# Mirko-Nava/BayesianNeuralNetworks

Measured on AMD Instinct MI355X. Metric: MC-samples/sec (node), 784-1200-1200-10 BayesianLinear MLP, batch 512, higher is better.
Workload: dtype bf16; 1 GPU; configs[1]: MNIST-shape 784-1200-1200-10 NormalLinear MLP, batch 512, 8 MC samples per forward per GPU (8 in all), KL once per forward, predictive mean; bf16 operands / fp32 accumulate; batch=512, hip_graph=True

## Files before the change

### bayesianneuralnetworks_amd/csrc/bnn_dense.hip

```cpp
#include <cstdlib>
#include <type_traits>

#include "bnn_device.hpp"
#include "bnn_dma.hpp"
#include "bnn_kl_body.hpp"

namespace bnn {

typedef float f32x4 __attribute__((ext_vector_type(4)));
typedef __bf16 bf16x8 __attribute__((ext_vector_type(8)));

constexpr int kDrawMaxTensors = 8;
constexpr int kDrawSpreadBelow = 4096;

struct DrawTensorDev {
    const float *mu;
    const float *rho;
    void *out;
    int64_t out_sample_stride;
    int32_t rows, cols, ld;
    int32_t bf16;
    int32_t kind;
    int32_t perm_taps;
    int32_t first_item;
// ... 207 lines not shown
        s_lo = local / nit;
        local -= s_lo * nit;
        s_hi = s_lo < S ? s_lo + 1 : 0;
        s_step = 1;
    }
    if (t_kind == 3) {
        if (L.t[ti].spread ? s_lo != 0 : blockIdx.y != 0) return;
        s_lo = 0; s_hi = 1; s_step = 1;
    }
    const int row = local / gpr, c0 = (local - row * gpr) << 3;
    if (row >= t_rows) return;
    const int64_t orow = (int64_t)row * t_ld + c0;
    const int esz = t_bf16 ? 2 : 4;
    char *const dst0 = t_out + orow * esz;
    const int64_t sbytes = t_stride * esz;
    const int64_t pbytes = sbytes * (t_kind == 3 ? 1 : L.nsamples);
    if (!LEAN && t_kind == BNN_DRAW_FLIPOUT) {
        float m[8], sg[8];
#pragma unroll
        for (int j = 0; j < 8; ++j) {
            const bool v = c0 + j < t_cols;
            m[j] = v ? t_mu[(int64_t)row * t_cols + c0 + j] : 0.f;
            sg[j] = v ? sigma_draw(t_rho[(int64_t)row * t_cols + c0 + j]) : 0.f;
        }
        const uint32_t edev = rng_epoch_dev(rng);
        const uint32_t e0 = (uint32_t)t_rows + (uint32_t)c0, q0 = e0 >> 2, off = e0 & 3u;
#pragma unroll 1
        for (int s = s_lo; s < s_hi; s += s_step) {
            const uint32_t sample = rng.sample0 + (uint32_t)s;
            const float r = flip_sign(drop_u1(rng, edev, (uint32_t)row, sample));
            const float4 ua = drop_u4(rng, edev, q0, sample), ub = drop_u4(rng, edev, q0 + 1u, sample), uc = drop_u4(rng, edev, q0 + 2u, sample);
            const float u[12] = {ua.x, ua.y, ua.z, ua.w, ub.x, ub.y, ub.z, ub.w, uc.x, uc.y, uc.z, uc.w};
            float w[8];
#pragma unroll
            for (int j = 0; j < 8; ++j) {
                const float uj = off == 0u ? u[j] : off == 1u ? u[j + 1] : off == 2u ? u[j + 2] : u[j + 3];
                w[j] = fmaf(sg[j], r * flip_sign(uj), m[j]);
            }
            char *dst = dst0 + (int64_t)s * sbytes;
            if (t_bf16) {
                uint4 o;
                o.x = pack_bf16x2(w[0], w[1]); o.y = pack_bf16x2(w[2], w[3]);
                o.z = pack_bf16x2(w[4], w[5]); o.w = pack_bf16x2(w[6], w[7]);
                *reinterpret_cast<uint4 *>(dst) = o;
            } else {
#pragma unroll
                for (int j = 0; j < 8; ++j)
                    if (c0 + j < t_ld) reinterpret_cast<float *>(dst)[j] = w[j];
            }
        }
        return;
    }
    const bool regular = t_bf16 && t_kind == 0 && t_taps <= 1 && (t_cols & 7) == 0 &&
                         (((reinterpret_cast<uintptr_t>(t_mu) | reinterpret_cast<uintptr_t>(t_rho)) & 15u) == 0);
    if (regular) {
        const bool pad = c0 >= t_cols;
        const int64_t e0 = pad ? 0 : (int64_t)row * t_cols + c0;
        const uint32_t edev = rng_epoch_dev(rng);
        const float4 m0 = *reinterpret_cast<const float4 *>(t_mu + e0), m1 = *reinterpret_cast<const float4 *>(t_mu + e0 + 4);
        const float4 r0 = *reinterpret_cast<const float4 *>(t_rho + e0), r1 = *reinterpret_cast<const float4 *>(t_rho + e0 + 4);
        const float live = pad ? 0.f : 1.f;
        const float m[8] = {pad ? 0.f : m0.x, pad ? 0.f : m0.y, pad ? 0.f : m0.z, pad ? 0.f : m0.w,
                            pad ? 0.f : m1.x, pad ? 0.f : m1.y, pad ? 0.f : m1.z, pad ? 0.f : m1.w};
        const float sg[8] = {live * sigma_draw(r0.x), live * sigma_draw(r0.y), live * sigma_draw(r0.z), live * sigma_draw(r0.w),
                             live * sigma_draw(r1.x), live * sigma_draw(r1.y), live * sigma_draw(r1.z), live * sigma_draw(r1.w)};
        const PhiloxKeys keys = philox_keys(rng.key0, rng.key1);
        const uint32_t blk = (uint32_t)(e0 >> 2);
        char *dst = dst0 + (int64_t)s_lo * sbytes;
        const int64_t step = sbytes * (int64_t)s_step;
        const bool gen16 = LEAN || rng.gen == BNN_GEN_PHILOX7_U16;
#pragma unroll U
        for (int s = s_lo; s < s_hi; s += s_step, dst += step) {
            const uint32_t sample = rng.sample0 + (uint32_t)s;
            float4 za, zb;
            if (gen16) {
                eps8_u16(rng, keys, edev, blk >> 1, sample, za, zb);
            } else {
                za = eps4(rng, keys, edev, blk, sample);
                zb = eps4(rng, keys, edev, blk + 1u, sample);
            }
            float w[8];
            w[0] = fmaf(sg[0], za.x, m[0]); w[1] = fmaf(sg[1], za.y, m[1]);
            w[2] = fmaf(sg[2], za.z, m[2]); w[3] = fmaf(sg[3], za.w, m[3]);
            w[4] = fmaf(sg[4], zb.x, m[4]); w[5] = fmaf(sg[5], zb.y, m[5]);
            w[6] = fmaf(sg[6], zb.z, m[6]); w[7] = fmaf(sg[7], zb.w, m[7]);
            if (t_x3) {
                uint4 h, mm, l;
                split_bf16x3(w[0], w[1], h.x, mm.x, l.x); split_bf16x3(w[2], w[3], h.y, mm.y, l.y);
                split_bf16x3(w[4], w[5], h.z, mm.z, l.z); split_bf16x3(w[6], w[7], h.w, mm.w, l.w);
                *reinterpret_cast<uint4 *>(dst) = h;
                *reinterpret_cast<uint4 *>(dst + pbytes) = mm;
                *reinterpret_cast<uint4 *>(dst + 2 * pbytes) = l;
            } else {
                uint4 o;
                o.x = pack_bf16x2(w[0], w[1]); o.y = pack_bf16x2(w[2], w[3]);
                o.z = pack_bf16x2(w[4], w[5]); o.w = pack_bf16x2(w[6], w[7]);
                *reinterpret_cast<uint4 *>(dst) = o;
            }
        }
        return;
    }
    if (LEAN) {
        const int64_t e0 = (int64_t)row * t_cols + c0;
        const int nval = c0 >= t_cols ? 0 : t_cols - c0 < 8 ? t_cols - c0 : 8;
        float m[8], sg[8];
#pragma unroll
        for (int j = 0; j < 8; ++j) {
            const bool v = j < nval;
            m[j] = v ? (t_kind != 2 ? t_mu[e0 + j] : sigma_accurate(t_rho[e0 + j])) : 0.f;
            sg[j] = v && t_kind == 0 ? sigma_draw(t_rho[e0 + j]) : 0.f;
        }
        const uint32_t edev = rng_epoch_dev(rng);
        const uint32_t blk = (uint32_t)(e0 >> 2);
        for (int s = s_lo; s < s_hi; s += s_step) {
            const uint32_t sample = rng.sample0 + (uint32_t)s;
            float4 za = make_float4(0.f, 0.f, 0.f, 0.f), zb = za;
            if (t_kind == 0) {
                za = eps4_u16(rng, edev, blk, sample);
                zb = eps4_u16(rng, edev, blk + 1u, sample);
            }
            float w[8];
            w[0] = fmaf(sg[0], za.x, m[0]); w[1] = fmaf(sg[1], za.y, m[1]);
            w[2] = fmaf(sg[2], za.z, m[2]); w[3] = fmaf(sg[3], za.w, m[3]);
            w[4] = fmaf(sg[4], zb.x, m[4]); w[5] = fmaf(sg[5], zb.y, m[5]);
            w[6] = fmaf(sg[6], zb.z, m[6]); w[7] = fmaf(sg[7], zb.w, m[7]);
#pragma unroll
            for (int j = 0; j < 8; ++j) w[j] = j < nval ? w[j] : 0.f;
            char *dst = dst0 + s * sbytes;
            if (t_bf16) {
                uint4 o;
                o.x = pack_bf16x2(w[0], w[1]); o.y = pack_bf16x2(w[2], w[3]);
                o.z = pack_bf16x2(w[4], w[5]); o.w = pack_bf16x2(w[6], w[7]);
                *reinterpret_cast<uint4 *>(dst) = o;
            } else {
#pragma unroll
                for (int j = 0; j < 8; ++j)
                    if (c0 + j < t_ld) reinterpret_cast<float *>(dst)[j] = w[j];
            }
        }
        return;
    }
    if (c0 >= t_cols) {
        for (int s = s_lo; s < s_hi; s += s_step) {
            if (t_bf16) {
                for (int pl = 0; pl < (t_x3 ? 3 : 1); ++pl) *reinterpret_cast<uint4 *>(dst0 + s * sbytes + pl * pbytes) = make_uint4(0u, 0u, 0u, 0u);
            } else
                for (int j = 0; j < 8; ++j)
                    if (c0 + j < t_ld) reinterpret_cast<float *>(dst0 + s * sbytes)[j] = 0.f;
        }
        return;
    }
    const int64_t e0 = (int64_t)row * t_cols + c0;
    const int nval = t_cols - c0 < 8 ? t_cols - c0 : 8;
    const bool full = nval == 8 && (((reinterpret_cast<uintptr_t>(t_mu) | reinterpret_cast<uintptr_t>(t_rho)) & 15u) == 0) && (e0 & 3) == 0;
    float m[8], sg[8];
    if (t_kind != 0) {
#pragma unroll
        for (int j = 0; j < 8; ++j) {
            m[j] = j < nval ? (t_kind != 2 ? t_mu[e0 + j] : sigma_accurate(t_rho[e0 + j])) : 0.f;
            sg[j] = 0.f;
        }
    } else if (full) {
        const float4 m0 = *reinterpret_cast<const float4 *>(t_mu + e0), m1 = *reinterpret_cast<const float4 *>(t_mu + e0 + 4);
        const float4 r0 = *reinterpret_cast<const float4 *>(t_rho + e0), r1 = *reinterpret_cast<const float4 *>(t_rho + e0 + 4);
        m[0] = m0.x; m[1] = m0.y; m[2] = m0.z; m[3] = m0.w; m[4] = m1.x; m[5] = m1.y; m[6] = m1.z; m[7] = m1.w;
        sg[0] = sigma_draw(r0.x); sg[1] = sigma_draw(r0.y); sg[2] = sigma_draw(r0.z); sg[3] = sigma_draw(r0.w);
        sg[4] = sigma_draw(r1.x); sg[5] = sigma_draw(r1.y); sg[6] = sigma_draw(r1.z); sg[7] = sigma_draw(r1.w);
    } else {
#pragma unroll
        for (int j = 0; j < 8; ++j) {
            m[j] = j < nval ? t_mu[e0 + j] : 0.f;
            sg[j] = j < nval ? sigma_draw(t_rho[e0 + j]) : 0.f;
        }
    }
    const uint32_t edev = rng_epoch_dev(rng);
    const PhiloxKeys keys = philox_keys(rng.key0, rng.key1);
    const uint32_t blk = (uint32_t)(e0 >> 2);
    const bool vec_store = t_bf16 && nval == 8 && t_taps <= 1;
#pragma unroll U
    for (int s = s_lo; s < s_hi; s += s_step) {
        const uint32_t sample = rng.sample0 + (uint32_t)s;
        float4 za = make_float4(0.f, 0.f, 0.f, 0.f), zb = za;
        if (LEAN && t_kind == 0) {
            za = eps4_u16(rng, keys, edev, blk, sample);
            zb = eps4_u16(rng, keys, edev, blk + 1u, sample);
        } else if (t_kind == 0) {
            za = eps4(rng, keys, edev, blk, sample);
            zb = eps4(rng, keys, edev, blk + 1u, sample);
        }
        float w[8];
        w[0] = fmaf(sg[0], za.x, m[0]); w[1] = fmaf(sg[1], za.y, m[1]);
        w[2] = fmaf(sg[2], za.z, m[2]); w[3] = fmaf(sg[3], za.w, m[3]);
        w[4] = fmaf(sg[4], zb.x, m[4]); w[5] = fmaf(sg[5], zb.y, m[5]);
        w[6] = fmaf(sg[6], zb.z, m[6]); w[7] = fmaf(sg[7], zb.w, m[7]);
        char *dst = dst0 + s * sbytes;
        if (vec_store && t_x3) {
            uint4 h, m, l;
            split_bf16x3(w[0], w[1], h.x, m.x, l.x); split_bf16x3(w[2], w[3], h.y, m.y, l.y);
            split_bf16x3(w[4], w[5], h.z, m.z, l.z); split_bf16x3(w[6], w[7], h.w, m.w, l.w);
            *reinterpret_cast<uint4 *>(dst) = h;
            *reinterpret_cast<uint4 *>(dst + pbytes) = m;
            *reinterpret_cast<uint4 *>(dst + 2 * pbytes) = l;
        } else if (vec_store) {
            uint4 o;
            o.x = pack_bf16x2(w[0], w[1]); o.y = pack_bf16x2(w[2], w[3]);
            o.z = pack_bf16x2(w[4], w[5]); o.w = pack_bf16x2(w[6], w[7]);
            *reinterpret_cast<uint4 *>(dst) = o;
        } else if (!LEAN && t_taps > 1) {
            const int Cn = t_cols / t_taps;
            uint16_t *rowp = reinterpret_cast<uint16_t *>(t_out + ((int64_t)row * t_ld) * 2 + s * sbytes);
            for (int j = 0; j < nval; ++j) {
                const int col = c0 + j, c = col / t_taps, tp = col - c * t_taps;
                if (t_x3) {
                    uint32_t h, m, l;
                    split_bf16x3(w[j], 0.f, h, m, l);
                    rowp[tp * Cn + c] = (uint16_t)h;
                    *reinterpret_cast<uint16_t *>(reinterpret_cast<char *>(rowp + tp * Cn + c) + pbytes) = (uint16_t)m;
                    *reinterpret_cast<uint16_t *>(reinterpret_cast<char *>(rowp + tp * Cn + c) + 2 * pbytes) = (uint16_t)l;
                } else
                    rowp[tp * Cn + c] = f2bf(w[j]);
            }
            for (int j = nval; j < 8 && c0 + j < t_ld; ++j)
                for (int pl = 0; pl < (t_x3 ? 3 : 1); ++pl)
                    *reinterpret_cast<uint16_t *>(reinterpret_cast<char *>(rowp + c0 + j) + pl * pbytes) = 0;
        } else {
            for (int j = 0; j < 8; ++j) {
                if (c0 + j >= t_ld) break;
                const float v = j < nval ? w[j] : 0.f;
                if (t_x3) {
                    uint32_t h, m, l;
                    split_bf16x3(v, 0.f, h, m, l);
                    reinterpret_cast<uint16_t *>(dst)[j] = (uint16_t)h;
                    reinterpret_cast<uint16_t *>(dst + pbytes)[j] = (uint16_t)m;
                    reinterpret_cast<uint16_t *>(dst + 2 * pbytes)[j] = (uint16_t)l;
                } else if (t_bf16) reinterpret_cast<uint16_t *>(dst)[j] = f2bf(v);
                else reinterpret_cast<float *>(dst)[j] = v;
            }
        }
    }
}

struct DenseParams {
    const uint16_t *A;
    int64_t a_sample_stride;
    int64_t lda;
    const uint16_t *W;
    int64_t w_sample_stride;
    int64_t ldw;
    const float *bias;
    int64_t bias_sample_stride;
    void *Y;
    int64_t y_sample_stride;
    int64_t ldy;
    int32_t M, N, K, S;
    int32_t ntm, ntn;
    int32_t flags;
    int32_t x3;
    int64_t a_plane_stride, w_plane_stride, y_plane_stride;
    const uint16_t *Wh;
    int64_t wh_sample_stride, ldwh;
    const float *bias_h;
    int64_t bias_h_sample_stride;
    float *P;
    int32_t Nh;
    int64_t wh_plane_stride;
    RngDev drop_rng;
    float drop_p, drop_scale;
    int32_t drop_fan;
};

constexpr int kDenseLoaderPrio = 1 << 21;
constexpr int kDenseNoXcdMap = 1 << 20;

__device__ __forceinline__ void dma_piece(const void *base, uint32_t voff, uint32_t lds)
{
    uint32_t keep;
    asm volatile("s_mov_b32 %0, m0\n\ts_mov_b32 m0, %3\n\ts_nop 0\n\tglobal_load_lds_dwordx4 %1, %2\n\ts_mov_b32 m0, %0"
                 : "=&s"(keep) : "v"(voff), "s"(base), "s"(lds) : "memory");
}

template <int TM, int TN, int NWM, int NWN, int ST, int YM, bool RELU, int DIAG = 0, bool DROP = false>
__global__ __launch_bounds__(512, ST == 2 ? 4 : 1) void k_dense_bf16(const DenseParams p)
{
    static_assert(!DROP || YM <= 1, "the dropout epilogue stores fp32 or bf16");
    constexpr bool CO = ST == 2;
    constexpr int NWV = 4;
    constexpr bool INTERLEAVE = true;
    constexpr int MPR = DIAG == 3 ? 1 : DIAG == 4 ? 2 : TN >= 8 ? 2 : 1;
    static_assert(NWM * NWN == NWV, "four consumer waves");
    constexpr int WM = 16 * TM, WN = 16 * TN, BM = NWM * WM, BN = NWN * WN;
    constexpr int A_TOTAL = BM / 8;
    constexpr int B_TOTAL = BN / 8;
    static_assert(A_TOTAL % NWV == 0, "A pieces divide evenly over the loaders");
    constexpr int A_PIECES = A_TOTAL / NWV;
    constexpr int B_BASE = B_TOTAL / NWV, B_EXTRA = B_TOTAL % NWV;
    constexpr int A_STAGE = BM * 128;
    constexpr int B_STAGE = BN * 128;
    constexpr int STAGE = A_STAGE + B_STAGE;
    constexpr bool YBF = YM != 0;
    constexpr int ESZ = YBF ? 2 : 4;
    constexpr int EPI_BYTES = ST * STAGE / NWV;
    constexpr int EPI_A = (EPI_BYTES / (16 * (WN * ESZ + 16))) < TM ? (EPI_BYTES / (16 * (WN * ESZ + 16))) : TM;
    static_assert(EPI_A >= 1, "a quarter of the ring must hold at least 16 output rows (epilogue staging)");
    __shared__ __attribute__((aligned(16))) char lds[ST * STAGE];

    const int per_s = p.ntm * p.ntn;
    int s, t;
    {
        const int L = (int)blockIdx.x;
        if (p.flags & kDenseNoXcdMap) {
            s = L / per_s;
            t = L % per_s;
        } else if (p.S % 8 == 0) {
            const int idx = L >> 3;
            s = (L & 7) + 8 * (idx / per_s);
            t = idx % per_s;
        } else {
            const int total = per_s * p.S, x = L & 7;
            const int u = x * (total >> 3) + (x < (total & 7) ? x : (total & 7)) + (L >> 3);
            s = u / per_s;
            t = u % per_s;
        }
    }
    int mt, panel;
    if (per_s > 32 && !(p.flags & kDenseNoXcdMap)) {
        constexpr int GM = 4;
        const int grp = t / (GM * p.ntn), first = grp * GM;
        const int gm = p.ntm - first < GM ? p.ntm - first : GM;
        const int v = t - grp * (GM * p.ntn);
        mt = first + v % gm;
        panel = v / gm;
    } else {
        mt = t / p.ntn;
        panel = t % p.ntn;
    }
    const int m0 = mt * BM, n0 = panel * BN;
    const int tid = threadIdx.x, lane = tid & 63;
    const int wave = __builtin_amdgcn_readfirstlane(tid >> 6);
    const int nk = (p.K + 63) / 64 * (p.x3 ? 6 : 1);

    if (wave >= NWV) {
        const int lw = wave - NWV;
        if (p.flags & kDenseLoaderPrio) __builtin_amdgcn_s_setprio(2);
        const uint32_t ring = __builtin_amdgcn_readfirstlane(lds_addr_of(lds));
        const int prow = lane >> 3;
        const int schunk = (lane & 7) ^ prow;
        const char *a_base = reinterpret_cast<const char *>(p.A + (int64_t)s * p.a_sample_stride);
        const char *w_base = reinterpret_cast<const char *>(p.W + (int64_t)s * p.w_sample_stride);
        uint32_t a_off[A_PIECES], b_off[B_BASE + 1];
        uint32_t a_dst[A_PIECES], b_dst[B_BASE + 1];
#pragma unroll
        for (int j = 0; j < A_PIECES; ++j) {
            const int r0 = (lw + NWV * j) * 8;
            int m = m0 + r0 + prow;
            m = m < p.M ? m : p.M - 1;
            a_off[j] = (uint32_t)((int64_t)m * p.lda * 2);
            a_dst[j] = (uint32_t)((r0 / WM) * (ST * WM * 128) + (r0 % WM) * 128);
        }
#pragma unroll
        for (int j = 0; j < B_BASE + 1; ++j) {
            const int r0 = (lw + NWV * j) * 8;
            int n = n0 + r0 + prow;
            n = n < p.N ? n : p.N - 1;
            b_off[j] = (uint32_t)((int64_t)n * p.ldw * 2) + 16u * (uint32_t)schunk;
            b_dst[j] = (uint32_t)(ST * A_STAGE + (r0 / WN) * (ST * WN * 128) + (r0 % WN) * 128);
        }
        const uint32_t a_colmax = (uint32_t)(p.K * 2 - 16);
        auto run = [&](auto nbp_c) {
            constexpr int NBP = decltype(nbp_c)::value;
            constexpr int P = A_PIECES + NBP;
            auto issue = [&](int kt) {
                if constexpr (DIAG == 2 || DIAG == 5 || DIAG == 8 || DIAG == 9) return;
                const int stage = kt % ST;
                int kb = kt;
                const char *ab = a_base, *wb = w_base;
                if (p.x3) {
                    const int nkb = (p.K + 63) >> 6;
                    int pr = 5;
                    if (kt < 5 * nkb) { kb = kt / 5; pr = kt - 5 * kb; } else kb = kt - 5 * nkb;
                    ab += ((0x001102 >> (4 * pr)) & 3) * (p.a_plane_stride * 2);
                    wb += ((0x010120 >> (4 * pr)) & 3) * (p.w_plane_stride * 2);
                }
                const uint32_t colA0 = (uint32_t)(kb * 128 + 16 * schunk);
                const uint32_t colA = colA0 < a_colmax ? colA0 : a_colmax;
                const uint32_t colB = (uint32_t)(kb * 128);
                const uint32_t sa = ring + (uint32_t)(stage * (WM * 128)), sb = ring + (uint32_t)(stage * (WN * 128));
#pragma unroll
                for (int j = 0; j < A_PIECES; ++j)
                    dma_piece(ab, a_off[j] + colA, sa + a_dst[j]);
#pragma unroll
                for (int j = 0; j < NBP; ++j)
                    dma_piece(wb, b_off[j] + colB, sb + b_dst[j]);
            };
#pragma unroll
            for (int i = 0; i < ST - 1; ++i)
                if (i < nk) issue(i);
            for (int kt = 0; kt < nk; ++kt) {
                const int ahead = nk - 1 - kt < ST - 2 ? nk - 1 - kt : ST - 2;
                if (ST >= 4 && ahead == 2) asm volatile("s_waitcnt vmcnt(%0)" :: "n"(2 * P) : "memory");
                else if (ahead >= 1) asm volatile("s_waitcnt vmcnt(%0)" :: "n"(P) : "memory");
                else asm volatile("s_waitcnt vmcnt(0)" ::: "memory");
                if constexpr (DIAG != 5 && DIAG != 9) __builtin_amdgcn_s_barrier();
                if (kt + ST - 1 < nk) issue(kt + ST - 1);
            }
            __builtin_amdgcn_s_barrier();
        };
        if (lw < B_EXTRA) run(std::integral_constant<int, B_BASE + 1>{});
        else run(std::integral_constant<int, B_BASE>{});
        return;
    }

    static_assert(ST == 2 || ST == 3 || ST == 4, "ring depth");
    uint64_t stamp[5] = {0, 0, 0, 0, 0};
    if constexpr (DIAG >= 6) stamp[0] = __builtin_amdgcn_s_memrealtime();
    const int fi = lane & 15, fq = lane >> 4;
    const int wm = wave / NWN, wn = wave % NWN;
    const char *a_rows = lds + wm * (ST * WM * 128);
    const char *b_rows = lds + ST * A_STAGE + wn * (ST * WN * 128);
    __builtin_amdgcn_s_setprio(1);
    f32x4 acc[TM][TN];
#pragma unroll
    for (int a = 0; a < TM; ++a)
#pragma unroll
        for (int b = 0; b < TN; ++b) acc[a][b] = f32x4{0.f, 0.f, 0.f, 0.f};
    const int fbase0 = fi * 128 + (((0 + fq) ^ (fi & 7)) << 4);
    const int fbase1 = fi * 128 + (((4 + fq) ^ (fi & 7)) << 4);
    uint4 fa[2][TM], fb[2][TN];
    auto rd = [&](auto buf_c, uint32_t stage, auto h_c) {
        constexpr int buf = decltype(buf_c)::value, h = decltype(h_c)::value;
        if constexpr (DIAG == 1 || DIAG == 7) return;
        const char *As = a_rows + (stage * (uint32_t)(WM * 128) + (uint32_t)(h ? fbase1 : fbase0));
        const char *Bs = b_rows + (stage * (uint32_t)(WN * 128) + (uint32_t)(h ? fbase1 : fbase0));
#pragma unroll
        for (int b = 0; b < TN; ++b) fb[buf][b] = *reinterpret_cast<const uint4 *>(Bs + b * 2048);
#pragma unroll
        for (int a = 0; a < TM; ++a) fa[buf][a] = *reinterpret_cast<const uint4 *>(As + a * 2048);
    };
    auto mm = [&](auto buf_c) {
        constexpr int buf = decltype(buf_c)::value;
        if constexpr (DIAG == 1 || DIAG == 7) return;
#pragma unroll
        for (int a = 0; a < TM; ++a)
#pragma unroll
            for (int b = 0; b < TN; ++b)
                acc[a][b] = __builtin_amdgcn_mfma_f32_16x16x32_bf16(__builtin_bit_cast(bf16x8, fb[buf][b]),
                                                                    __builtin_bit_cast(bf16x8, fa[buf][a]), acc[a][b], 0, 0, 0);
    };
    using I0 = std::integral_constant<int, 0>;
    using I1 = std::integral_constant<int, 1>;
    auto interleave = [&]() {
        if constexpr ((DIAG == 0 || (DIAG >= 3 && DIAG != 7)) && INTERLEAVE) {
            constexpr int NI = (TM * TN) / MPR < TM + TN ? (TM * TN) / MPR : TM + TN;
#pragma unroll
            for (int i = 0; i < NI; ++i) {
                __builtin_amdgcn_sched_group_barrier(0x008, MPR, 0);
                __builtin_amdgcn_sched_group_barrier(0x100, 1, 0);
            }
            if constexpr (TM + TN > NI) __builtin_amdgcn_sched_group_barrier(0x100, TM + TN - NI, 0);
            if constexpr (TM * TN > MPR * NI) __builtin_amdgcn_sched_group_barrier(0x008, TM * TN - MPR * NI, 0);
        }
    };
    auto first_half = [&](uint32_t stage) {
        rd(I1{}, stage, I1{});
        if constexpr (!INTERLEAVE) __builtin_amdgcn_sched_barrier(0);
        mm(I0{});
        interleave();
        __builtin_amdgcn_sched_barrier(0);
    };
    auto second_half = [&](uint32_t next) {
        asm volatile("s_waitcnt lgkmcnt(0)" ::: "memory");
        if constexpr (DIAG != 5 && DIAG != 9) __builtin_amdgcn_s_barrier();
        asm volatile("" ::: "memory");
        rd(I0{}, next, I0{});
        if constexpr (!INTERLEAVE) __builtin_amdgcn_sched_barrier(0);
        mm(I1{});
        interleave();
        __builtin_amdgcn_sched_barrier(0);
    };
    const float *bias = p.bias ? p.bias + (int64_t)s * p.bias_sample_stride : nullptr;
    const int mw = m0 + wm * WM, nw = n0 + wn * WN;
    constexpr bool BIAS_PRE = TM * TN <= 20 && !CO;
    float bv[TN][4];
    auto load_bias = [&]() {
#pragma unroll
        for (int b = 0; b < TN; ++b)
#pragma unroll
            for (int r = 0; r < 4; ++r) {
                const int n = nw + b * 16 + fq * 4 + r;
                bv[b][r] = (bias && n < p.N) ? bias[n] : 0.f;
            }
    };
    if constexpr (BIAS_PRE) load_bias();
    const uint32_t drop_ed = DROP ? rng_epoch_dev(p.drop_rng) : 0u;
    if (DIAG == 0 && (nw >= p.N || mw >= p.M)) {
        for (int kt = 0; kt < nk + 1; ++kt) __builtin_amdgcn_s_barrier();
        if constexpr (YM == 3) {
            float *P = p.P + ((int64_t)(panel * NWN + wn) * p.S + s) * (int64_t)p.M * p.Nh;
            for (int i = lane; i < WM * p.Nh; i += 64) {
                const int m = mw + i / p.Nh;
                if (m < p.M) P[(int64_t)m * p.Nh + (i % p.Nh)] = 0.f;
            }
        }
        return;
    }
    if constexpr (DIAG != 5 && DIAG != 9) __builtin_amdgcn_s_barrier();
    asm volatile("" ::: "memory");
    if constexpr (DIAG >= 6) stamp[1] = __builtin_amdgcn_s_memrealtime();
    if constexpr (CO) {
        uint32_t stage = 0;
        for (int kt = 0; kt + 1 < nk; ++kt) {
            rd(I0{}, stage, I0{});
            mm(I0{});
            __builtin_amdgcn_sched_barrier(0);
            rd(I0{}, stage, I1{});
            asm volatile("s_waitcnt lgkmcnt(0)" ::: "memory");
            if constexpr (DIAG != 5 && DIAG != 9) __builtin_amdgcn_s_barrier();
            asm volatile("" ::: "memory");
            mm(I0{});
            __builtin_amdgcn_sched_barrier(0);
            stage = stage + 1 == (uint32_t)ST ? 0u : stage + 1;
        }
        rd(I0{}, stage, I0{});
        mm(I0{});
        __builtin_amdgcn_sched_barrier(0);
        rd(I0{}, stage, I1{});
        mm(I0{});
    } else {
        rd(I0{}, 0u, I0{});
        uint32_t stage = 0;
        for (int kt = 0; kt + 1 < nk; ++kt) {
            const uint32_t next = stage + 1 == (uint32_t)ST ? 0u : stage + 1;
            first_half(stage);
            second_half(next);
            stage = next;
        }
        first_half(stage);
        mm(I1{});
    }
    __builtin_amdgcn_sched_barrier(0);
    __builtin_amdgcn_s_setprio(0);
    asm volatile("s_waitcnt lgkmcnt(0)" ::: "memory");
    __builtin_amdgcn_s_barrier();
    asm volatile("" ::: "memory");
    if constexpr (DIAG >= 6) stamp[2] = __builtin_amdgcn_s_memrealtime();
    auto leave_stamps = [&]() {
        if constexpr (DIAG >= 6) {
            stamp[3] = __builtin_amdgcn_s_memrealtime();
            asm volatile("s_waitcnt vmcnt(0)" ::: "memory");
            stamp[4] = __builtin_amdgcn_s_memrealtime();
            if (wave == 0 && lane == 0 && p.P) {
                uint64_t *q = reinterpret_cast<uint64_t *>(p.P) + (int64_t)blockIdx.x * 5;
                for (int i = 0; i < 5; ++i) q[i] = stamp[i];
            }
        }
    };

    if constexpr (!BIAS_PRE) load_bias();
    constexpr bool BIAS_IN_ACC = CO && !DROP;
    if constexpr (BIAS_IN_ACC) {
#pragma unroll
        for (int a = 0; a < TM; ++a)
#pragma unroll
            for (int b = 0; b < TN; ++b)
#pragma unroll
                for (int r = 0; r < 4; ++r) acc[a][b][r] += bv[b][r];
    }
    if constexpr (DROP) {
#pragma unroll
        for (int a = 0; a < TM; ++a)
#pragma unroll
            for (int b = 0; b < TN; ++b)
#pragma unroll
                for (int r = 0; r < 4; ++r) {
                    float v = acc[a][b][r] + bv[b][r];
                    if (RELU) v = fmaxf(v, 0.f);
                    acc[a][b][r] = v * p.drop_scale;
                }
    }
    auto vals = [&](int a, int b, float (&v)[4], int so = 0) {
        if constexpr (DROP) {
            uint32_t q = ((uint32_t)(mw + a * 16 + fi) * (uint32_t)p.N + (uint32_t)(nw + b * 16 + fq * 4)) >> 2;
            RngDev rk = p.drop_rng;
            asm volatile("" : "+v"(q), "+s"(rk.key0), "+s"(rk.key1));
            const float4 u4 = drop_u4(rk, drop_ed, q, p.drop_rng.sample0 + (uint32_t)so);
            const float u[4] = {u4.x, u4.y, u4.z, u4.w};
#pragma unroll
            for (int r = 0; r < 4; ++r) v[r] = (u[r] < p.drop_p || p.drop_scale == 0.f) ? 0.f : acc[a][b][r];
        } else {
#pragma unroll
            for (int r = 0; r < 4; ++r) {
                v[r] = BIAS_IN_ACC ? acc[a][b][r] : acc[a][b][r] + bv[b][r];
                if (RELU) v[r] = fmaxf(v[r], 0.f);
            }
        }
    };
    if constexpr (YM == 3) {
        constexpr bool X3_HEAD_FITS = 3 * WM * (WN * 2 + 16) <= EPI_BYTES;
        if constexpr (X3_HEAD_FITS) if (p.x3) {
            constexpr int pitch = WN * 2 + 16;
            char *T = lds + wave * EPI_BYTES;
#pragma unroll
            for (int a = 0; a < TM; ++a)
#pragma unroll
                for (int b = 0; b < TN; ++b) {
                    float v[4];
                    vals(a, b, v);
                    uint32_t h0, m0, l0, h1, m1, l1;
                    split_bf16x3(v[0], v[1], h0, m0, l0);
                    split_bf16x3(v[2], v[3], h1, m1, l1);
                    char *q = T + (a * 16 + fi) * pitch + (b * 16 + fq * 4) * 2;
                    *reinterpret_cast<uint2 *>(q) = make_uint2(h0, h1);
                    *reinterpret_cast<uint2 *>(q + WM * pitch) = make_uint2(m0, m1);
                    *reinterpret_cast<uint2 *>(q + 2 * WM * pitch) = make_uint2(l0, l1);
                }
            __builtin_amdgcn_fence(__ATOMIC_RELEASE, "workgroup");
            __builtin_amdgcn_wave_barrier();
            const int Nh = p.Nh;
            const int hrow = fi < Nh ? fi : Nh - 1;
            const uint16_t *wh = p.Wh + (int64_t)s * p.wh_sample_stride + (int64_t)hrow * p.ldwh;
            f32x4 hacc[TM], hsm[TM];
#pragma unroll
            for (int a = 0; a < TM; ++a) { hacc[a] = f32x4{0.f, 0.f, 0.f, 0.f}; hsm[a] = hacc[a]; }
            constexpr int NC = (WN + 31) / 32;
#pragma unroll
            for (int c = 0; c < NC; ++c) {
                const int kcol = 32 * c + 8 * fq;
                const int n = nw + kcol;
                const bool okb = kcol < WN && fi < Nh && n + 8 <= (int)p.ldwh;
                uint4 bf[3];
#pragma unroll
                for (int pl = 0; pl < 3; ++pl)
                    bf[pl] = okb ? *reinterpret_cast<const uint4 *>(wh + pl * p.wh_plane_stride + n) : make_uint4(0u, 0u, 0u, 0u);
#pragma unroll
                for (int a = 0; a < TM; ++a) {
                    uint4 af[3];
#pragma unroll
                    for (int pl = 0; pl < 3; ++pl)
                        af[pl] = kcol < WN ? *reinterpret_cast<const uint4 *>(T + pl * WM * pitch + (a * 16 + fi) * pitch + kcol * 2) : make_uint4(0u, 0u, 0u, 0u);
                    auto mf = [&](f32x4 c4, int pa, int pw) {
                        return __builtin_amdgcn_mfma_f32_16x16x32_bf16(__builtin_bit_cast(bf16x8, af[pa]), __builtin_bit_cast(bf16x8, bf[pw]), c4, 0, 0, 0);
                    };
                    hsm[a] = mf(mf(mf(mf(mf(hsm[a], 2, 0), 0, 2), 1, 1), 1, 0), 0, 1);
                    hacc[a] = mf(hacc[a], 0, 0);
                }
            }
            const int part = panel * NWN + wn;
            float hb = 0.f;
            if (part == 0 && p.bias_h && fi < Nh) hb = p.bias_h[(int64_t)s * p.bias_h_sample_stride + fi];
            float *P = p.P + ((int64_t)part * p.S + s) * (int64_t)p.M * Nh;
#pragma unroll
            for (int a = 0; a < TM; ++a)
#pragma unroll
                for (int r = 0; r < 4; ++r) {
                    const int m = mw + a * 16 + fq * 4 + r;
                    if (m < p.M && fi < Nh) P[(int64_t)m * Nh + fi] = (hacc[a][r] + hsm[a][r]) + hb;
                }
            return;
        }
        constexpr int pitch = WN * 2 + 16;
        static_assert(WM * pitch <= EPI_BYTES, "the wave's quarter of the ring holds its bf16 tile");
        char *T = lds + wave * EPI_BYTES;
#pragma unroll
        for (int a = 0; a < TM; ++a)
#pragma unroll
            for (int b = 0; b < TN; ++b) {
                float v[4];
                vals(a, b, v);
                *reinterpret_cast<uint2 *>(T + (a * 16 + fi) * pitch + (b * 16 + fq * 4) * 2) = make_uint2(pack_bf16x2(v[0], v[1]), pack_bf16x2(v[2], v[3]));
            }
        __builtin_amdgcn_fence(__ATOMIC_RELEASE, "workgroup");
        __builtin_amdgcn_wave_barrier();
        const int Nh = p.Nh;
        const int hrow = fi < Nh ? fi : Nh - 1;
        const uint16_t *wh = p.Wh + (int64_t)s * p.wh_sample_stride + (int64_t)hrow * p.ldwh;
        f32x4 hacc[TM];
#pragma unroll
        for (int a = 0; a < TM; ++a) hacc[a] = f32x4{0.f, 0.f, 0.f, 0.f};
        constexpr int NC = (WN + 31) / 32;
#pragma unroll
        for (int c = 0; c < NC; ++c) {
            const int kcol = 32 * c + 8 * fq;
            const int n = nw + kcol;
            uint4 bf = make_uint4(0u, 0u, 0u, 0u);
            if (kcol < WN && fi < Nh && n + 8 <= (int)p.ldwh) bf = *reinterpret_cast<const uint4 *>(wh + n);
#pragma unroll
            for (int a = 0; a < TM; ++a) {
                uint4 af = make_uint4(0u, 0u, 0u, 0u);
                if (kcol < WN) af = *reinterpret_cast<const uint4 *>(T + (a * 16 + fi) * pitch + kcol * 2);
                hacc[a] = __builtin_amdgcn_mfma_f32_16x16x32_bf16(__builtin_bit_cast(bf16x8, af), __builtin_bit_cast(bf16x8, bf), hacc[a], 0, 0, 0);
            }
        }
        const int part = panel * NWN + wn;
        float hb = 0.f;
        if (part == 0 && p.bias_h && fi < Nh) hb = p.bias_h[(int64_t)s * p.bias_h_sample_stride + fi];
        float *P = p.P + ((int64_t)part * p.S + s) * (int64_t)p.M * Nh;
#pragma unroll
        for (int a = 0; a < TM; ++a)
#pragma unroll
            for (int r = 0; r < 4; ++r) {
                const int m = mw + a * 16 + fq * 4 + r;
                if (m < p.M && fi < Nh) P[(int64_t)m * Nh + fi] = hacc[a][r] + hb;
            }
        return;
    }
    auto plane_of = [&](float v, int pl) -> uint16_t {
        const uint16_t h = f2bf(v);
        if (pl == 0) return h;
        const float r = v - __uint_as_float((uint32_t)h << 16);
        const uint16_t m = f2bf(r);
        if (pl == 1) return m;
        return f2bf(r - __uint_as_float((uint32_t)m << 16));
    };
    constexpr int NP = YM == 2 ? 3 : 1;
    const int ncopy = DROP ? p.drop_fan : 1;
    const bool wide = nw + WN <= p.N && mw + WM <= p.M && (p.ldy * ESZ) % 16 == 0 && (nw * ESZ) % 16 == 0 &&
                      ((reinterpret_cast<uintptr_t>(p.Y) + (int64_t)s * p.y_sample_stride * ESZ) & 15u) == 0 &&
                      (NP == 1 || (p.y_plane_stride * ESZ) % 16 == 0) && (!DROP || ncopy == 1 || (p.y_sample_stride * ESZ) % 16 == 0);
    for (int cp = 0; cp < ncopy; ++cp) {
    const int so = s + cp;
    const int64_t ybase = (int64_t)so * p.y_sample_stride * ESZ;
    if (wide) {
        char *T = lds + wave * EPI_BYTES;
        constexpr int row_bytes = WN * ESZ;
        constexpr int pitch = row_bytes + 16;
        constexpr int cpr = row_bytes / 16;
#pragma unroll
        for (int pl = 0; pl < NP; ++pl) {
            char *Y8 = reinterpret_cast<char *>(p.Y) + ybase + ((int64_t)pl * p.y_plane_stride + (int64_t)mw * p.ldy + nw) * ESZ;
#pragma unroll
            for (int a0 = 0; a0 < TM; a0 += EPI_A) {
#pragma unroll
                for (int b = 0; b < TN; ++b)
#pragma unroll
                    for (int a = a0; a < a0 + EPI_A && a < TM; ++a) {
                        float v[4];
                        vals(a, b, v, so);
                        char *q = T + ((a - a0) * 16 + fi) * pitch + (b * 16 + fq * 4) * ESZ;
                        if (YM == 2)
                            *reinterpret_cast<uint2 *>(q) = make_uint2((uint32_t)plane_of(v[0], pl) | ((uint32_t)plane_of(v[1], pl) << 16),
                                                                       (uint32_t)plane_of(v[2], pl) | ((uint32_t)plane_of(v[3], pl) << 16));
                        else if (YM == 1) *reinterpret_cast<uint2 *>(q) = make_uint2(pack_bf16x2(v[0], v[1]), pack_bf16x2(v[2], v[3]));
                        else *reinterpret_cast<float4 *>(q) = make_float4(v[0], v[1], v[2], v[3]);
                    }
                __builtin_amdgcn_fence(__ATOMIC_RELEASE, "workgroup");
                __builtin_amdgcn_wave_barrier();
                const int nrows = (TM - a0 < EPI_A ? TM - a0 : EPI_A) * 16;
                for (int c = lane; c < nrows * cpr; c += 64) {
                    const int row = c / cpr, cc = c - row * cpr;
                    *reinterpret_cast<uint4 *>(Y8 + (int64_t)(a0 * 16 + row) * p.ldy * ESZ + cc * 16) =
                        *reinterpret_cast<const uint4 *>(T + row * pitch + cc * 16);
                }
                __builtin_amdgcn_fence(__ATOMIC_RELEASE, "workgroup");
                __builtin_amdgcn_wave_barrier();
            }
        }
        continue;
    }
    float *Yf = reinterpret_cast<float *>(p.Y) + (int64_t)so * p.y_sample_stride;
    uint16_t *Yh = reinterpret_cast<uint16_t *>(p.Y) + (int64_t)so * p.y_sample_stride;
#pragma unroll
    for (int a = 0; a < TM; ++a) {
        const int m = mw + a * 16 + fi;
        if (m >= p.M) continue;
#pragma unroll
        for (int b = 0; b < TN; ++b) {
            float v[4];
            vals(a, b, v, so);
#pragma unroll
            for (int r = 0; r < 4; ++r) {
                const int n = nw + b * 16 + fq * 4 + r;
                if (n >= p.N) continue;
                if (YM == 2) {
#pragma unroll
                    for (int pl = 0; pl < 3; ++pl) Yh[(int64_t)pl * p.y_plane_stride + (int64_t)m * p.ldy + n] = plane_of(v[r], pl);
                } else if (YM == 1) Yh[(int64_t)m * p.ldy + n] = f2bf(v[r]);
                else Yf[(int64_t)m * p.ldy + n] = v[r];
            }
        }
    }
    }
    if (wide) leave_stamps();
}

constexpr int kHeadMaxSteps = 16;

__global__ __launch_bounds__(256) void k_head_bf16(const DenseParams p)
{
    __shared__ float red[4][16][17];
    const int ntm = p.ntm;
    const int s = (int)blockIdx.x / ntm, mt = (int)blockIdx.x % ntm;
    const int tid = threadIdx.x, lane = tid & 63, wave = tid >> 6;
    const int fi = lane & 15, fq = lane >> 4;
    const int nk = (p.K + 31) / 32;
    const int per = (nk + 3) / 4;
    const int k0 = wave * per, k1 = (k0 + per < nk) ? k0 + per : nk;
    int m = mt * 16 + fi;
    m = m < p.M ? m : p.M - 1;
    int n = fi < p.N ? fi : p.N - 1;
    const uint16_t *arow = p.A + (int64_t)s * p.a_sample_stride + (int64_t)m * p.lda;
    const uint16_t *wrow = p.W + (int64_t)s * p.w_sample_stride + (int64_t)n * p.ldw;
    uint4 af[kHeadMaxSteps], bfr[kHeadMaxSteps];
    const int kmax = p.K - 8;
    f32x4 acc = f32x4{0.f, 0.f, 0.f, 0.f};
    const int npass = p.x3 ? 6 : 1;
    for (int pass = 0; pass < npass; ++pass) {
        const uint16_t *ar = arow, *wr = wrow;
        if (p.x3) {
            ar += ((0x001102 >> (4 * pass)) & 3) * p.a_plane_stride;
            wr += ((0x010120 >> (4 * pass)) & 3) * p.w_plane_stride;
        }
#pragma unroll
        for (int i = 0; i < kHeadMaxSteps; ++i) {
            const int kt = k0 + i;
            int ka = kt * 32 + 8 * fq;
            const int kb = ka;
            ka = ka < kmax ? ka : kmax;
            if (kt < k1) {
                af[i] = *reinterpret_cast<const uint4 *>(ar + ka);
                bfr[i] = *reinterpret_cast<const uint4 *>(wr + kb);
            } else {
                af[i] = make_uint4(0u, 0u, 0u, 0u);
                bfr[i] = make_uint4(0u, 0u, 0u, 0u);
            }
        }
#pragma unroll
        for (int i = 0; i < kHeadMaxSteps; ++i)
            acc = __builtin_amdgcn_mfma_f32_16x16x32_bf16(__builtin_bit_cast(bf16x8, af[i]), __builtin_bit_cast(bf16x8, bfr[i]), acc, 0, 0, 0);
    }
#pragma unroll
    for (int r = 0; r < 4; ++r) red[wave][fq * 4 + r][fi] = acc[r];
    __syncthreads();
    const int row = tid >> 4, col = tid & 15;
    const int mo = mt * 16 + row;
    if (mo < p.M && col < p.N) {
        float v = ((red[0][row][col] + red[1][row][col]) + red[2][row][col]) + red[3][row][col];
        if (p.bias) v += p.bias[(int64_t)s * p.bias_sample_stride + col];
        if (p.flags & BNN_FLAG_RELU) v = fmaxf(v, 0.f);
        if (p.flags & BNN_FLAG_Y_BF16) reinterpret_cast<uint16_t *>(p.Y)[(int64_t)s * p.y_sample_stride + (int64_t)mo * p.ldy + col] = f2bf(v);
        else reinterpret_cast<float *>(p.Y)[(int64_t)s * p.y_sample_stride + (int64_t)mo * p.ldy + col] = v;
    }
}

struct ConvParams {
    const float *X;
    int64_t x_sample_stride;
    const uint16_t *W;
    int64_t w_sample_stride;
    int64_t ldw;
    const float *bias;
    int64_t bias_sample_stride;
    float *Y;
    int64_t y_sample_stride;
    int32_t B, C, H, Wd, O, KH, KW, sh, sw, ph, pw, dh, dw, OH, OW;
    int32_t S, IMG, ntiles;
    int32_t img_bytes;
    int32_t flags;
    const float *sgn_in;
    const float *sgn_out;
    int64_t w_plane_stride;
    RngDev rng;
};

constexpr int kConvLds = 78 * 1024;
constexpr int kConvLdsBig = 136 * 1024;

template <int TN, int ST, int LDSB, bool FLIP = false, bool X3 = false, int NS = 0>
__global__ __launch_bounds__(512, LDSB <= 80 * 1024 ? 2 : 1) void k_conv_bf16(const ConvParams p)
{
    constexpr bool KEYED = NS > 0;
    static_assert(!KEYED || (FLIP && !X3), "keyed signs: the bf16 Flipout launch");
    constexpr int NSX = KEYED ? NS : 1;
    constexpr int TO = FLIP ? TN / 2 : TN;
    constexpr int NACC = FLIP ? TO * (1 + NSX) : TN;
    constexpr int NWV = 4, TM = 2, WM = 32, BN = 16 * TN;
    constexpr int B_TOTAL = BN / 8, NBP = B_TOTAL / NWV;
    constexpr int B_STAGE = BN * 128;
    static_assert(B_TOTAL % NWV == 0, "B pieces split evenly over the loaders");
    static_assert(ST >= 2 && ST * B_STAGE < LDSB, "ring");
    __shared__ __attribute__((aligned(16))) char lds[LDSB];
    const int P = p.OH * p.OW, HW = p.H * p.Wd;
    const int CPX = p.C >> 3;
    const int mask_stride = FLIP ? p.IMG * CPX * 16 : 0;
    const int mask_region = mask_stride * NSX;
    const int img_region = p.IMG * p.img_bytes;
    constexpr int NPL = X3 ? 3 : 1;
    char *masks = lds + NPL * img_region;
    char *b_ring = lds + NPL * img_region + mask_region;
    constexpr int NOUT = FLIP ? BN / 2 : BN;

    int s, t;
    const int SG = KEYED ? (p.S + NSX - 1) / NSX : p.S;
    {
        const int L = (int)blockIdx.x;
        if (SG % 8 == 0) { const int idx = L >> 3; s = (L & 7) + 8 * (idx / p.ntiles); t = idx % p.ntiles; }
        else { s = L / p.ntiles; t = L % p.ntiles; }
    }
    if constexpr (KEYED) s *= NSX;
    const int nvalid = KEYED ? (p.S - s < NSX ? p.S - s : NSX) : 1;
    const int b0 = t * p.IMG;
    const int imgs = (p.B - b0 < p.IMG) ? p.B - b0 : p.IMG;
    const int tid = threadIdx.x, lane = tid & 63;
    const int wave = __builtin_amdgcn_readfirstlane(tid >> 6);
    const bool swz16 = (p.C >> 3) >= 16;
    auto swz = [&](int pl) { return swz16 ? (pl & 15) : ((pl >> 1) & 7); };
    const int nkb = p.KH * p.KW * (p.C >> 6);
    const int nk = nkb * (X3 ? 6 : 1);

    const int lw = wave - NWV;
    uint32_t b_off[NBP];
    uint32_t b_lds = 0;
    const char *w_base = reinterpret_cast<const char *>(p.W + (int64_t)s * p.w_sample_stride);
    auto issue = [&](int kt) {
        const int stage = kt % ST;
        int kb = kt;
        const char *wb = w_base;
        if constexpr (X3) {
            int pr = 5;
            if (kt < 5 * nkb) { kb = kt / 5; pr = kt - 5 * kb; } else kb = kt - 5 * nkb;
            wb += ((0x010120 >> (4 * pr)) & 3) * (p.w_plane_stride * 2);
        }
#pragma unroll
        for (int j = 0; j < NBP; ++j)
            dma_piece(wb, b_off[j] + (uint32_t)(kb * 128), b_lds + (uint32_t)(stage * B_STAGE + (lw + NWV * j) * 1024));
    };
    if (wave >= NWV) {
        b_lds = __builtin_amdgcn_readfirstlane(lds_addr_of(b_ring));
        const int prow = lane >> 3, schunk = (lane & 7) ^ prow;
#pragma unroll
        for (int j = 0; j < NBP; ++j) {
            int n = (lw + NWV * j) * 8 + prow;
            const int nrows = FLIP ? 2 * p.O : p.O;
            n = n < nrows ? n : nrows - 1;
            b_off[j] = (uint32_t)((int64_t)n * p.ldw * 2) + 16u * (uint32_t)schunk;
        }
#pragma unroll
        for (int k0 = 0; k0 < ST - 1; ++k0)
            if (k0 < nk) issue(k0);
    }

    {
        const float *xs = p.X + (int64_t)s * p.x_sample_stride + (int64_t)b0 * p.C * HW;
        const int Q = (HW + 3) >> 2, CH2 = p.C >> 1;
        const int per_img = (p.flags & 1) ? 0 : CH2 * Q;
        if constexpr (KEYED) {
            const uint32_t ed = rng_epoch_dev(p.rng);
            const uint32_t row_w = (uint32_t)(p.O + p.C);
            float *rs = reinterpret_cast<float *>(lds + LDSB) - NSX * p.IMG * p.O;
            for (int i = tid; i < NSX * imgs * CPX; i += 512) {
                const int n = i / (imgs * CPX), r = i - n * imgs * CPX, il = r / CPX, ch = r - il * CPX;
                uint32_t w4[4] = {0u, 0u, 0u, 0u};
                if (n < nvalid) {
                    const uint32_t smp = p.rng.sample0 + (uint32_t)(s + n);
                    const uint32_t e0 = (uint32_t)(b0 + il) * row_w + (uint32_t)p.O + 8u * (uint32_t)ch;
                    const float4 ua = drop_u4(p.rng, ed, e0 >> 2, smp), ub = drop_u4(p.rng, ed, (e0 >> 2) + 1u, smp);
                    const float u[8] = {ua.x, ua.y, ua.z, ua.w, ub.x, ub.y, ub.z, ub.w};
#pragma unroll
                    for (int j = 0; j < 4; ++j)
                        w4[j] = (flip_sign(u[2 * j]) < 0.f ? 0x8000u : 0u) | (flip_sign(u[2 * j + 1]) < 0.f ? 0x80000000u : 0u);
                }
                *reinterpret_cast<uint4 *>(masks + n * mask_stride + (il * CPX + ch) * 16) = make_uint4(w4[0], w4[1], w4[2], w4[3]);
            }
            const int OQ = p.O >> 2;
            for (int i = tid; i < NSX * imgs * OQ; i += 512) {
                const int n = i / (imgs * OQ), r = i - n * imgs * OQ, il = r / OQ, q = r - il * OQ;
                float4 v = make_float4(1.f, 1.f, 1.f, 1.f);
                if (n < nvalid) {
                    const uint32_t smp = p.rng.sample0 + (uint32_t)(s + n);
                    const uint32_t e0 = (uint32_t)(b0 + il) * row_w + 4u * (uint32_t)q;
                    const float4 u = drop_u4(p.rng, ed, e0 >> 2, smp);
                    v = make_float4(flip_sign(u.x), flip_sign(u.y), flip_sign(u.z), flip_sign(u.w));
                }
                *reinterpret_cast<float4 *>(rs + (n * p.IMG + il) * p.O + 4 * q) = v;
            }
        } else if constexpr (FLIP) {
            for (int i = tid; i < imgs * CPX; i += 512) {
                const int il = i / CPX, ch = i - il * CPX;
                const float *sp = p.sgn_in + (int64_t)(b0 + il) * p.C + ch * 8;
                uint32_t w4[4];
#pragma unroll
                for (int j = 0; j < 4; ++j)
                    w4[j] = (sp[2 * j] < 0.f ? 0x8000u : 0u) | (sp[2 * j + 1] < 0.f ? 0x80000000u : 0u);
                *reinterpret_cast<uint4 *>(masks + i * 16) = make_uint4(w4[0], w4[1], w4[2], w4[3]);
            }
        }
        const bool vec = (HW & 3) == 0 && ((reinterpret_cast<uintptr_t>(xs) & 15u) == 0);
        const int img_elems = p.C * HW;
        for (int rem = tid; rem < per_img; rem += 512) {
            const int cp = rem / Q, q = rem - cp * Q;
            int dst[4];
#pragma unroll
            for (int j = 0; j < 4; ++j) {
                const int pl = 4 * q + j;
                dst[j] = pl < HW ? pl * (p.C * 2) + (((cp >> 2) ^ swz(pl)) << 4) + (cp & 3) * 4 : -1;
            }
            const float *g0 = xs + (int64_t)(2 * cp) * HW + 4 * q;
            constexpr int UB = 8;
            for (int il = 0; il < imgs; il += UB) {
// ... 843 lines not shown
```

Measured before the change: 228,400 MC-samples/s.

## Prefetch bias and head weights into LDS in the loader wave; skip out-of-range DMA

In the co-resident (CO) dense kernel, the loader waves now prefetch the bias vector and the fused-head weight tile into a side region of LDS before the main loop. The consumer epilogue then reads them from LDS instead of global memory. Loaders also skip DMA pieces for rows past the M/N edge, zero-filling those LDS slots once instead. The last half-k MFMA step is skipped when K's tail fits in the first half. This removes global-load latency from the epilogue and wasted edge traffic, at the cost of extra LDS per workgroup and a vmcnt(0) wait in the loader prologue.

```diff
diff --git a/bayesianneuralnetworks_amd/csrc/bnn_dense.hip b/bayesianneuralnetworks_amd/csrc/bnn_dense.hip
--- a/bayesianneuralnetworks_amd/csrc/bnn_dense.hip
+++ b/bayesianneuralnetworks_amd/csrc/bnn_dense.hip
@@ -533,7 +533,16 @@
     constexpr int EPI_BYTES = ST * STAGE / NWV;
     constexpr int EPI_A = (EPI_BYTES / (16 * (WN * ESZ + 16))) < TM ? (EPI_BYTES / (16 * (WN * ESZ + 16))) : TM;
     static_assert(EPI_A >= 1, "a quarter of the ring must hold at least 16 output rows (epilogue staging)");
-    __shared__ __attribute__((aligned(16))) char lds[ST * STAGE];
+#ifndef BNN_CO_SIDE
+#define BNN_CO_SIDE 1
+#endif
+    constexpr bool SIDE = CO && BNN_CO_SIDE;
+    constexpr int HW_PITCH = BN * 2 + 16;
+    constexpr int SIDE_NF = BN + (YM == 3 ? 16 : 0);
+    constexpr int SIDE_BIAS = ST * STAGE, SIDE_HEAD = SIDE_BIAS + SIDE_NF * 4;
+    constexpr int SIDE_BYTES = !SIDE ? 0 : SIDE_NF * 4 + (YM == 3 ? 16 * HW_PITCH : 0);
+    static_assert(!CO || ST * STAGE + SIDE_BYTES <= 80 * 1024, "two co-resident workgroups share the CU's 160 KiB of LDS");
+    __shared__ __attribute__((aligned(16))) char lds[ST * STAGE + SIDE_BYTES];
 
     const int per_s = p.ntm * p.ntn;
     int s, t;
@@ -597,6 +606,62 @@
             b_dst[j] = (uint32_t)(ST * A_STAGE + (r0 / WN) * (ST * WN * 128) + (r0 % WN) * 128);
         }
         const uint32_t a_colmax = (uint32_t)(p.K * 2 - 16);
+        int na = A_PIECES, nb = B_BASE + 1;
+        if constexpr (CO) {
+            const int va = ((p.M - m0 < BM ? p.M - m0 : BM) + 7) >> 3, vb = ((p.N - n0 < BN ? p.N - n0 : BN) + 7) >> 3;
+            na = (va - lw + NWV - 1) / NWV;
+            nb = (vb - lw + NWV - 1) / NWV;
+            na = __builtin_amdgcn_readfirstlane(na < A_PIECES ? na : A_PIECES);
+            nb = __builtin_amdgcn_readfirstlane(nb < B_BASE + 1 ? nb : B_BASE + 1);
+            const uint4 z = make_uint4(0u, 0u, 0u, 0u);
+#pragma unroll
+            for (int j = 0; j < A_PIECES; ++j)
+                if (j >= na) {
+#pragma unroll
+                    for (int i = 0; i < ST; ++i) *reinterpret_cast<uint4 *>(lds + i * (WM * 128) + a_dst[j] + 16 * lane) = z;
+                }
+#pragma unroll
+            for (int j = 0; j < B_BASE + 1; ++j)
+                if (j >= nb && lw + NWV * j < B_TOTAL) {
+#pragma unroll
+                    for (int i = 0; i < ST; ++i) *reinterpret_cast<uint4 *>(lds + i * (WN * 128) + b_dst[j] + 16 * lane) = z;
+                }
+        }
+        const int lt = lw * 64 + lane;
+        constexpr int CPR = BN / 8, NU = (16 * CPR + 255) / 256;
+        float sbv = 0.f;
+        uint4 hv[NU];
+        auto side_request = [&]() {
+            const float *bias_l = p.bias ? p.bias + (int64_t)s * p.bias_sample_stride : nullptr;
+            const float *src = nullptr;
+            if (lt < BN) {
+                if (bias_l && n0 + lt < p.N) src = bias_l + (n0 + lt);
+            } else if (YM == 3 && lt < SIDE_NF) {
+                if (panel == 0 && p.bias_h && lt - BN < p.Nh) src = p.bias_h + ((int64_t)s * p.bias_h_sample_stride + (lt - BN));
+            }
+            if (src) sbv = *src;
+            if constexpr (YM == 3) {
+                const uint16_t *wh = p.Wh + (int64_t)s * p.wh_sample_stride;
+#pragma unroll
+                for (int u = 0; u < NU; ++u) {
+                    const int c = lt + 256 * u, row = c / CPR, n = n0 + (c - row * CPR) * 8;
+                    hv[u] = make_uint4(0u, 0u, 0u, 0u);
+                    if (row < p.Nh && n + 8 <= (int)p.ldwh) hv[u] = *reinterpret_cast<const uint4 *>(wh + (int64_t)row * p.ldwh + n);
+                }
+            }
+        };
+        auto side_store = [&]() {
+            asm volatile("s_waitcnt vmcnt(0)" ::: "memory");
+            if (lt < SIDE_NF) reinterpret_cast<float *>(lds + SIDE_BIAS)[lt] = sbv;
+            if constexpr (YM == 3) {
+#pragma unroll
+                for (int u = 0; u < NU; ++u) {
+                    const int c = lt + 256 * u, row = c / CPR;
+                    if (row < 16) *reinterpret_cast<uint4 *>(lds + SIDE_HEAD + row * HW_PITCH + (c - row * CPR) * 16) = hv[u];
+                }
+            }
+            asm volatile("s_waitcnt lgkmcnt(0)" ::: "memory");
+        };
         auto run = [&](auto nbp_c) {
             constexpr int NBP = decltype(nbp_c)::value;
             constexpr int P = A_PIECES + NBP;
@@ -618,14 +683,16 @@
                 const uint32_t sa = ring + (uint32_t)(stage * (WM * 128)), sb = ring + (uint32_t)(stage * (WN * 128));
 #pragma unroll
                 for (int j = 0; j < A_PIECES; ++j)
-                    dma_piece(ab, a_off[j] + colA, sa + a_dst[j]);
+                    if (!CO || j < na) dma_piece(ab, a_off[j] + colA, sa + a_dst[j]);
 #pragma unroll
                 for (int j = 0; j < NBP; ++j)
-                    dma_piece(wb, b_off[j] + colB, sb + b_dst[j]);
+                    if (!CO || j < nb) dma_piece(wb, b_off[j] + colB, sb + b_dst[j]);
             };
+            if constexpr (SIDE) side_request();
 #pragma unroll
             for (int i = 0; i < ST - 1; ++i)
                 if (i < nk) issue(i);
+            if constexpr (SIDE) side_store();
             for (int kt = 0; kt < nk; ++kt) {
                 const int ahead = nk - 1 - kt < ST - 2 ? nk - 1 - kt : ST - 2;
                 if (ST >= 4 && ahead == 2) asm volatile("s_waitcnt vmcnt(%0)" :: "n"(2 * P) : "memory");
@@ -713,6 +780,14 @@
     constexpr bool BIAS_PRE = TM * TN <= 20 && !CO;
     float bv[TN][4];
     auto load_bias = [&]() {
+        if constexpr (SIDE) {
+#pragma unroll
+            for (int b = 0; b < TN; ++b) {
+                const float4 v = *reinterpret_cast<const float4 *>(lds + SIDE_BIAS + (wn * WN + b * 16 + fq * 4) * 4);
+                bv[b][0] = v.x; bv[b][1] = v.y; bv[b][2] = v.z; bv[b][3] = v.w;
+            }
+            return;
+        }
 #pragma unroll
         for (int b = 0; b < TN; ++b)
 #pragma unroll
@@ -754,8 +829,10 @@
         rd(I0{}, stage, I0{});
         mm(I0{});
         __builtin_amdgcn_sched_barrier(0);
-        rd(I0{}, stage, I1{});
-        mm(I0{});
+        if (p.x3 || ((p.K - 1) & 63) >= 32) {
+            rd(I0{}, stage, I1{});
+            mm(I0{});
+        }
     } else {
         rd(I0{}, 0u, I0{});
         uint32_t stage = 0;
@@ -913,7 +990,9 @@
             const int kcol = 32 * c + 8 * fq;
             const int n = nw + kcol;
             uint4 bf = make_uint4(0u, 0u, 0u, 0u);
-            if (kcol < WN && fi < Nh && n + 8 <= (int)p.ldwh) bf = *reinterpret_cast<const uint4 *>(wh + n);
+            if constexpr (SIDE) {
+                if (kcol < WN) bf = *reinterpret_cast<const uint4 *>(lds + SIDE_HEAD + fi * HW_PITCH + (wn * WN + kcol) * 2);
+            } else if (kcol < WN && fi < Nh && n + 8 <= (int)p.ldwh) bf = *reinterpret_cast<const uint4 *>(wh + n);
 #pragma unroll
             for (int a = 0; a < TM; ++a) {
                 uint4 af = make_uint4(0u, 0u, 0u, 0u);
@@ -923,7 +1002,9 @@
         }
         const int part = panel * NWN + wn;
         float hb = 0.f;
-        if (part == 0 && p.bias_h && fi < Nh) hb = p.bias_h[(int64_t)s * p.bias_h_sample_stride + fi];
+        if constexpr (SIDE) {
+            if (part == 0) hb = reinterpret_cast<const float *>(lds + SIDE_BIAS)[BN + fi];
+        } else if (part == 0 && p.bias_h && fi < Nh) hb = p.bias_h[(int64_t)s * p.bias_h_sample_stride + fi];
         float *P = p.P + ((int64_t)part * p.S + s) * (int64_t)p.M * Nh;
 #pragma unroll
         for (int a = 0; a < TM; ++a)
```

Result: slower. 217,300 MC-samples/s (-4.9%).
